# raulmur/ORB_SLAM2

Hardware: NVIDIA H100
Metric: stereo frames/sec (ORB extract L+R + ComputeStereoMatches, KITTI-shaped 1242x375 @2000 kpts) (higher is better)
Workload: dtype u8

## Files before the change

### orb_slam2_b200/csrc/k_fast.cu

```cuda
#include <cuda.h>

#include <cstring>

#include "borb_internal.h"

#include <algorithm>
#include <type_traits>
#include <vector>

namespace borb {

namespace {

constexpr int TP = 160;
constexpr int HB = FAST_H_BAND;
static_assert(HB >= 60 && HB <= 127, "a one-row band (hCell <= 59) must fit; collect packs the row into 7 bits");
constexpr int TROWS = HB + 6;
constexpr int QCAP = HB * 128;
constexpr int RG_MAX = (HB + 7) / 8;
constexpr int WSEG = RG_MAX * 32;
constexpr int RMAX = HB / 30;
constexpr int NCX = 128 / 30 + 1;
constexpr int SM_SCORE = TROWS * TP, SM_QUEUE = SM_SCORE + HB * TP, SM_WQUEUE = SM_QUEUE + QCAP * 2;
constexpr int FAST_SMEM = SM_WQUEUE + 8 * WSEG * 4;
static_assert(SM_SCORE % 16 == 0 && SM_WQUEUE % 4 == 0, "shared-memory carve-up alignment");

__device__ __forceinline__ uint32_t smem_u32(const void* p) { return (uint32_t)__cvta_generic_to_shared(p); }

template <int DX>
__device__ __forceinline__ uint32_t win(uint32_t W0, uint32_t W1, uint32_t W2) {
    if (DX == 0) return W1;
    if (DX > 0) return __byte_perm(W1, W2, DX | ((DX + 1) << 4) | ((DX + 2) << 8) | ((DX + 3) << 12));
    constexpr int K = 4 + DX;
    return __byte_perm(W0, W1, K | ((K + 1) << 4) | ((K + 2) << 8) | ((K + 3) << 12));
}

__device__ __forceinline__ uint32_t gt_flag(uint32_t q, uint32_t v, uint32_t K) {
    const uint32_t a = __vabsdiffu4(q, v);
    return (a + K) | a;
}

__device__ __forceinline__ uint32_t score_pair(const uint32_t (&d)[16], uint32_t v2) {
    uint32_t lo3[16], hi3[16];
#pragma unroll
    for (int k = 0; k < 16; k++) {
        lo3[k] = __vimin3_s16x2(d[k], d[(k + 1) & 15], d[(k + 2) & 15]);
        hi3[k] = __vimax3_s16x2(d[k], d[(k + 1) & 15], d[(k + 2) & 15]);
    }
    uint32_t lo9[16], hi9[16];
#pragma unroll
    for (int k = 0; k < 16; k++) {
        lo9[k] = __vimin3_s16x2(lo3[k], lo3[(k + 3) & 15], lo3[(k + 6) & 15]);
        hi9[k] = __vimax3_s16x2(hi3[k], hi3[(k + 3) & 15], hi3[(k + 6) & 15]);
    }
    uint32_t bb[5], dd[5];
#pragma unroll
    for (int k = 0; k < 5; k++) {
        bb[k] = __vimax3_s16x2(lo9[3 * k], lo9[3 * k + 1], lo9[3 * k + 2]);
        dd[k] = __vimin3_s16x2(hi9[3 * k], hi9[3 * k + 1], hi9[3 * k + 2]);
    }
    const uint32_t bright = __vimax3_s16x2(__vimax3_s16x2(bb[0], bb[1], bb[2]), __vimax3_s16x2(bb[3], bb[4], lo9[15]), bb[0]);
    const uint32_t darkm = __vimin3_s16x2(__vimin3_s16x2(dd[0], dd[1], dd[2]), __vimin3_s16x2(dd[3], dd[4], hi9[15]), dd[0]);
    return __viaddmax_s16x2_relu(__vmaxs2(__vsub2(bright, v2), __vsub2(v2, darkm)), 0xFFFFFFFFu, 0u);
}

__device__ __forceinline__ uint32_t score_pixels(const uint8_t* pa, const uint8_t* pb) {
    constexpr int RX[16] = {0, 1, 2, 3, 3, 3, 2, 1, 0, -1, -2, -3, -3, -3, -2, -1};
    constexpr int RY[16] = {3, 3, 2, 1, 0, -1, -2, -3, -3, -3, -2, -1, 0, 1, 2, 3};
    uint32_t d[16];
#pragma unroll
    for (int k = 0; k < 16; k++) {
        const int o = RY[k] * TP + RX[k];
        d[k] = (uint32_t)pa[o] | ((uint32_t)pb[o] << 16);
    }
    return score_pair(d, (uint32_t)pa[0] | ((uint32_t)pb[0] << 16));
}

}

struct TMaps { CUtensorMap m[BORB_MAX_LEVELS]; };

struct __align__(16) FastTile { int8_t l, ncell, rowsPerBlk, pad; int16_t x0, x1, y0, y1, wCell, hCell; };
static_assert(sizeof(FastTile) == 16, "one 16-byte load per CTA");

__global__ void __launch_bounds__(256, 4) fast_kernel(const __grid_constant__ Geometry g, const __grid_constant__ TMaps tm,
                                                   const FastTile* __restrict__ tiles, uint32_t* __restrict__ cand, int* __restrict__ cand_cnt) {
    extern __shared__ __align__(128) uint8_t smem[];
    uint8_t* tile = smem;
    uint8_t* score = smem + SM_SCORE;
    uint16_t* queue = reinterpret_cast<uint16_t*>(smem + SM_QUEUE);
    uint32_t* wqueue = reinterpret_cast<uint32_t*>(smem + SM_WQUEUE);
    __shared__ __align__(8) unsigned long long bar;
    __shared__ int pn, qn, needB;
    __shared__ int cellHasIni[RMAX * NCX];
    __shared__ uint8_t cellOf[128];
    __shared__ uint8_t rowOf[HB];

    const int img = blockIdx.y;
    const FastTile T = tiles[blockIdx.x];
    const int l = T.l, ncell = T.ncell, x0 = T.x0, x1 = T.x1, y0 = T.y0, y1 = T.y1;
    const int wCell = T.wCell, hCell = T.hCell;
    const LevelGeom& L = g.lv[l];
    const int tw = x1 - x0, th = y1 - y0;
    const int tid = threadIdx.x;
    const int lane = tid & 31, wrp = tid >> 5;

    const int xs = (x0 - 4) & ~15;
    const int off = x0 - xs;
    if (tid == 0) {
        asm volatile("mbarrier.init.shared::cta.b64 [%0], 1;" ::"r"(smem_u32(&bar)));
        asm volatile("fence.mbarrier_init.release.cluster;" ::: "memory");
        const uint32_t bytes = (uint32_t)TP * (uint32_t)fast_box_rows(T.rowsPerBlk, hCell);
        asm volatile("mbarrier.arrive.expect_tx.shared::cta.b64 _, [%0], %1;" ::"r"(smem_u32(&bar)), "r"(bytes) : "memory");
        asm volatile(
            "cp.async.bulk.tensor.3d.shared::cluster.global.tile.mbarrier::complete_tx::bytes [%0], [%1, {%2, %3, %4}], [%5];"
            ::"r"(smem_u32(tile)), "l"(reinterpret_cast<uint64_t>(&tm.m[l])), "r"(xs), "r"(y0 - 3), "r"(img), "r"(smem_u32(&bar))
            : "memory");
    }
    if (tid < RMAX * NCX) cellHasIni[tid] = 0;
    if (tid < 128) cellOf[tid] = (uint8_t)(tid / wCell);
    if (tid < HB) rowOf[tid] = (uint8_t)(tid / hCell);
    if (tid == 0) { pn = 0; qn = 0; needB = 0; }
    __syncthreads();
    asm volatile(
        "{\n"
        ".reg .pred p;\n"
        "FAST_TMA_WAIT:\n"
        "mbarrier.try_wait.parity.shared::cta.b64 p, [%0], 0;\n"
        "@p bra FAST_TMA_DONE;\n"
        "bra FAST_TMA_WAIT;\n"
        "FAST_TMA_DONE:\n"
        "}\n" ::"r"(smem_u32(&bar))
        : "memory");
    if (g.fast_mode == 1) {
        if (reinterpret_cast<const uint32_t*>(tile)[tid] == 0x12345678u && cand_cnt[0] == -1) cand[0] = 1;
        return;
    }

    const uint32_t* T32 = reinterpret_cast<const uint32_t*>(tile);
    uint32_t* S32 = reinterpret_cast<uint32_t*>(score);
    const int wbase = off >> 2;
    const int wc = wbase + lane;
    uint32_t vmask = 0;
#pragma unroll
    for (int b = 0; b < 4; b++)
        if (4 * wc + b - off >= 0 && 4 * wc + b - off < tw) vmask |= 0x80u << (8 * b);

    auto collect = [&](int t, const uint32_t (&mr)[RMAX], bool zero, auto banded) {
        constexpr bool BANDED = decltype(banded)::value;
        const uint32_t K = (uint32_t)(127 - min(t, 127)) * 0x01010101u;
        uint32_t mm[RMAX];
#pragma unroll
        for (int r = 0; r < (BANDED ? RMAX : 1); r++) {
            mm[r] = mr[r];
            asm volatile("" : "+r"(mm[r]));
        }
        const bool reject = t <= 127;
        const int RG = (th + 7) >> 3;
        const int yBeg = wrp * RG, yEnd = min(th, yBeg + RG);
        uint32_t a0[7], a1[7], a2[7];
        int wcount = 0;
        if (yBeg < yEnd) {
#pragma unroll
            for (int j = 0; j < 6; j++) {
                const uint32_t* rp = T32 + (yBeg + j) * (TP / 4) + wc - 1;
                a0[j] = rp[0]; a1[j] = rp[1]; a2[j] = rp[2];
            }
        }
        for (int it0 = 0; it0 < RG; it0 += 7)
#pragma unroll
        for (int it = 0; it < 7; it++) {
            const int yy = yBeg + it0 + it;
            if (yy < yEnd) {
                {
                    const uint32_t* rp = T32 + (yy + 6) * (TP / 4) + wc - 1;
                    a0[(it + 6) % 7] = rp[0]; a1[(it + 6) % 7] = rp[1]; a2[(it + 6) % 7] = rp[2];
                }
                uint32_t m = mm[0];
                if constexpr (BANDED) {
#pragma unroll
                    for (int r = 1; r < RMAX; r++)
                        if (yy >= r * hCell) m = mm[r];
                }
#define ROW(dy) a0[(it + (dy) + 3) % 7], a1[(it + (dy) + 3) % 7], a2[(it + (dy) + 3) % 7]
                uint32_t f = m;
                if (reject && m) {
                    const uint32_t v = a1[(it + 3) % 7];
                    uint32_t acc = gt_flag(win<0>(ROW(3)), v, K) | gt_flag(win<0>(ROW(-3)), v, K);
                    acc &= gt_flag(win<2>(ROW(2)), v, K) | gt_flag(win<-2>(ROW(-2)), v, K);
                    acc &= gt_flag(win<3>(ROW(0)), v, K) | gt_flag(win<-3>(ROW(0)), v, K);
                    acc &= gt_flag(win<2>(ROW(-2)), v, K) | gt_flag(win<-2>(ROW(2)), v, K);
                    f = acc & m;
                }
#undef ROW
                const unsigned bal = __ballot_sync(0xFFFFFFFFu, f != 0);
                if (zero && m != 0) S32[yy * (TP / 4) + wc] = 0;
                if (f) wqueue[wrp * WSEG + wcount + __popc(bal & ((1u << lane) - 1))] = f | (uint32_t)(yy << 8) | (uint32_t)wc;
                wcount += __popc(bal);
            }
        }
        __syncwarp();
        for (int i = 0; i < wcount; i += 32) {
            const uint32_t we = i + lane < wcount ? wqueue[wrp * WSEG + i + lane] : 0u;
            const uint32_t fl = we & 0x80808080u;
            const int c = __popc(fl);
            int incl = c;
#pragma unroll
            for (int o2 = 1; o2 < 32; o2 <<= 1) {
                const int s = __shfl_up_sync(0xFFFFFFFFu, incl, o2);
                if (lane >= o2) incl += s;
            }
            int base = 0;
            if (lane == 31) base = atomicAdd(&pn, incl);
            base = __shfl_sync(0xFFFFFFFFu, base, 31) + incl - c;
            const int e = (int)((we >> 8) & 127) << 8 | (int)(4 * (we & 127));
#pragma unroll
            for (int b = 0; b < 4; b++)
                if (fl & (0x80u << (8 * b))) queue[base++] = (uint16_t)(e + b);
        }
    };

    auto score_queue = [&](int t) {
        const int np = pn;
        const int tc = max(t, 1);
        for (int rb = 0; rb < np; rb += 512) {
            const int e0 = rb + wrp * 64 + lane, e1 = e0 + 32;
            const bool va = e0 < np, vb = e1 < np;
            const int qa = va ? queue[e0] : off;
            const int qb = vb ? queue[e1] : qa;
            __syncthreads();
            if (rb + wrp * 64 < np) {
                const int ia = (qa >> 8) * TP + (qa & 255), ib = (qb >> 8) * TP + (qb & 255);
                const uint32_t s2 = score_pixels(tile + ia + 3 * TP, tile + ib + 3 * TP);
                const int sa = (int)(s2 & 0xFFFFu), sb = (int)(s2 >> 16);
                if (va) score[ia] = (uint8_t)sa;
                if (vb) score[ib] = (uint8_t)sb;
                const bool ca = va && sa >= tc, cb = vb && sb >= tc;
                if (__any_sync(0xFFFFFFFFu, ca || cb)) {
                    const int c = (int)ca + (int)cb;
                    int incl = c;
#pragma unroll
                    for (int o2 = 1; o2 < 32; o2 <<= 1) {
                        const int s = __shfl_up_sync(0xFFFFFFFFu, incl, o2);
                        if (lane >= o2) incl += s;
                    }
                    int base = 0;
                    if (lane == 31) base = atomicAdd(&qn, incl);
                    base = __shfl_sync(0xFFFFFFFFu, base, 31) + incl - c;
                    if (ca) queue[base++] = (uint16_t)qa;
                    if (cb) queue[base] = (uint16_t)qb;
                }
            }
        }
    };

    {
        const uint32_t mA[RMAX] = {vmask};
        collect(g.ini_th, mA, true, std::false_type());
    }
    __syncthreads();
    if (g.fast_mode == 2) {
        if (pn == -1) cand[0] = 1;
        return;
    }
    score_queue(g.ini_th);
    __syncthreads();
    int nq = qn;
    if (g.fast_mode == 3) {
        if (nq == -1) cand[0] = 1;
        return;
    }

    uint32_t* out = cand + (size_t)img * g.cand_image_stride + L.cand_off;
    int* cnt = cand_cnt + img * g.nlevels + l;

    auto nms = [&](int n, bool mark) {
        for (int e = tid; e < n; e += 256) {
            const int q = queue[e];
            const int col = q & 255, yy = q >> 8;
            const int xx = col - off;
            const int s = score[yy * TP + col];
            const int c = cellOf[xx], r = rowOf[yy];
            const int cx0 = c * wCell, cx1 = min(cx0 + wCell, tw);
            const int cy0 = r * hCell, cy1 = min(cy0 + hCell, th);
            bool ismax = true;
#pragma unroll
            for (int dy = -1; dy <= 1; dy++)
#pragma unroll
                for (int dx = -1; dx <= 1; dx++) {
                    if (dx == 0 && dy == 0) continue;
                    const int qx = xx + dx, qy = yy + dy;
                    if (qx < cx0 || qx >= cx1 || qy < cy0 || qy >= cy1) continue;
                    if (!(s > (int)score[qy * TP + col + dx])) ismax = false;
                }
            if (ismax) {
                if (mark) cellHasIni[r * NCX + c] = 1;
            } else
                queue[e] = 0xFFFF;
        }
    };
    auto emit = [&](int n) {
        for (int eb = 0; eb < n; eb += 256) {
            const int e = eb + tid;
            int s = 0, xx = 0, yy = 0;
            if (e < n) {
                const int q = queue[e];
                if (q != 0xFFFF) {
                    const int col = q & 255;
                    yy = q >> 8; xx = col - off;
                    s = score[yy * TP + col];
                }
            }
            const unsigned m = __ballot_sync(0xFFFFFFFFu, s > 0);
            if (m) {
                int base = 0;
                if (lane == 0) base = atomicAdd(cnt, __popc(m));
                base = __shfl_sync(0xFFFFFFFFu, base, 0);
                if (s > 0) {
                    const int pos = base + __popc(m & ((1u << lane) - 1));
                    if (pos < L.cand_cap) out[pos] = pack_xys(x0 + xx, y0 + yy, s);
                }
            }
        }
    };

    nms(nq, true);
    __syncthreads();
    emit(nq);
    if (tid < RMAX * NCX) {
        const int r = tid / NCX, c = tid - r * NCX;
        if (r * hCell < th && c < ncell && c * wCell < tw && !cellHasIni[tid] && g.min_th < g.ini_th) needB = 1;
    }
    __syncthreads();
    if (!needB) return;

    {
        uint32_t need[RMAX];
#pragma unroll
        for (int r = 0; r < RMAX; r++) {
            need[r] = 0;
#pragma unroll
            for (int b = 0; b < 4; b++) {
                const int xx = 4 * wc + b - off;
                if (xx >= 0 && xx < tw && !cellHasIni[r * NCX + cellOf[xx]]) need[r] |= 0x80u << (8 * b);
            }
        }
        if (tid == 0) { pn = 0; qn = 0; }
        __syncthreads();
        collect(g.min_th, need, false, std::true_type());
        __syncthreads();
        score_queue(g.min_th);
        __syncthreads();
        nq = qn;
        nms(nq, false);
        __syncthreads();
        emit(nq);
    }
}

typedef CUresult (*EncodeTiledFn)(CUtensorMap*, CUtensorMapDataType, cuuint32_t, void*, const cuuint64_t*, const cuuint64_t*,
                                  const cuuint32_t*, const cuuint32_t*, CUtensorMapInterleave, CUtensorMapSwizzle,
                                  CUtensorMapL2promotion, CUtensorMapFloatOOBfill);

borb_status build_fast_tmaps(const Geometry& g, const Workspace& ws, void* out_tmaps) {
    static EncodeTiledFn encode = nullptr;
    if (!encode) {
        void* fn = nullptr;
        cudaDriverEntryPointQueryResult qres;
        cudaError_t e = cudaGetDriverEntryPoint("cuTensorMapEncodeTiled", &fn, cudaEnableDefault, &qres);
        if (e != cudaSuccess || qres != cudaDriverEntryPointSuccess || !fn) {
            set_error("cuTensorMapEncodeTiled unavailable (%s)", cudaGetErrorString(e));
            return BORB_ERR_CUDA;
        }
        encode = (EncodeTiledFn)fn;
    }
    TMaps* tm = reinterpret_cast<TMaps*>(out_tmaps);
    std::memset(tm, 0, sizeof(TMaps));
    for (int l = 0; l < g.nlevels; l++) {
        const LevelGeom& L = g.lv[l];
        cuuint64_t dims[3] = {(cuuint64_t)L.w, (cuuint64_t)L.h, (cuuint64_t)ws.max_images};
        cuuint64_t strides[2] = {(cuuint64_t)L.pitch, (cuuint64_t)g.pyr_image_stride};
        cuuint32_t box[3] = {(cuuint32_t)TP, (cuuint32_t)fast_box_rows(L.rowsPerBlk, L.hCell), 1};
        cuuint32_t estr[3] = {1, 1, 1};
        CUresult r = encode(&tm->m[l], CU_TENSOR_MAP_DATA_TYPE_UINT8, 3, ws.pyr + L.pyr_off, dims, strides, box, estr,
                            CU_TENSOR_MAP_INTERLEAVE_NONE, CU_TENSOR_MAP_SWIZZLE_NONE, CU_TENSOR_MAP_L2_PROMOTION_L2_128B,
                            CU_TENSOR_MAP_FLOAT_OOB_FILL_NONE);
        if (r != CUDA_SUCCESS) {
            set_error("cuTensorMapEncodeTiled failed for level %d (CUresult %d)", l, (int)r);
            return BORB_ERR_CUDA;
        }
    }
    return BORB_OK;
}

size_t fast_tmaps_bytes() { return sizeof(TMaps); }

borb_status build_fast_tiles(const Geometry& g, Workspace& ws) {
    std::vector<FastTile> t;
    for (int l = 0; l < g.nlevels; l++) {
        const LevelGeom& L = g.lv[l];
        for (int cellRow = 0; cellRow < L.nRows; cellRow += L.rowsPerBlk)
            for (int blkCol = 0; blkCol < L.blkCols; blkCol++) {
                const int cell0 = blkCol * L.cellsPerBlk;
                const int ncell = std::min(L.cellsPerBlk, L.nCols - cell0);
                const int nrow = std::min(L.rowsPerBlk, L.nRows - cellRow);
                const int x0 = EDGE + cell0 * L.wCell, x1 = std::min(x0 + ncell * L.wCell, L.w - EDGE);
                const int y0 = EDGE + cellRow * L.hCell, y1 = std::min(y0 + nrow * L.hCell, L.h - EDGE);
                if (x0 >= x1 || y0 >= y1) continue;
                FastTile f;
                f.l = (int8_t)l; f.ncell = (int8_t)ncell; f.rowsPerBlk = (int8_t)L.rowsPerBlk; f.pad = 0;
                f.x0 = (int16_t)x0; f.x1 = (int16_t)x1; f.y0 = (int16_t)y0; f.y1 = (int16_t)y1;
                f.wCell = (int16_t)L.wCell; f.hCell = (int16_t)L.hCell;
                t.push_back(f);
            }
    }
    cudaFree(ws.fast_tiles); ws.fast_tiles = nullptr;
    ws.fast_n_tiles = (int)t.size();
    if (t.empty()) return BORB_OK;
    BORB_CUDA(cudaMalloc(&ws.fast_tiles, t.size() * sizeof(FastTile)));
    BORB_CUDA(cudaMemcpy(ws.fast_tiles, t.data(), t.size() * sizeof(FastTile), cudaMemcpyHostToDevice));
    return BORB_OK;
}

int launch_fast(const Geometry& g, const Workspace& ws, int n_images, cudaStream_t s) {
    if (ws.fast_n_tiles == 0) return 0;
    allow_max_smem((const void*)fast_kernel);
    dim3 grid(ws.fast_n_tiles, n_images);
    fast_kernel<<<grid, 256, FAST_SMEM, s>>>(g, *reinterpret_cast<const TMaps*>(ws.fast_tmaps), reinterpret_cast<const FastTile*>(ws.fast_tiles), ws.cand, ws.cand_cnt);
    return 1;
}

}
```

Before: 44120.

## Process two FAST rows per step, warp-skip empty bands, fuse NMS and emit

The FAST collect loop now handles two rows per iteration in the unbanded pass and writes paired queue entries with 8-byte stores. The banded pass skips rows where no lane has a live mask. The score buffer is zeroed up front with vector stores, replacing the per-row zeroing inside collect. NMS now counts the survivors it keeps, so emit needs only one warp-level atomic per warp and drops one block barrier. In exchange it uses more registers and a larger wqueue segment, and emit now relies on each warp's NMS and emit covering the same entries.

Result: faster. 45390 (median of 6 runs) (+2.9%).

```diff
diff --git a/orb_slam2_b200/csrc/k_fast.cu b/orb_slam2_b200/csrc/k_fast.cu
--- a/orb_slam2_b200/csrc/k_fast.cu
+++ b/orb_slam2_b200/csrc/k_fast.cu
@@ -18,12 +18,12 @@
 constexpr int TROWS = HB + 6;
 constexpr int QCAP = HB * 128;
 constexpr int RG_MAX = (HB + 7) / 8;
-constexpr int WSEG = RG_MAX * 32;
+constexpr int WSEG = (RG_MAX + 1) / 2 * 64;
 constexpr int RMAX = HB / 30;
 constexpr int NCX = 128 / 30 + 1;
 constexpr int SM_SCORE = TROWS * TP, SM_QUEUE = SM_SCORE + HB * TP, SM_WQUEUE = SM_QUEUE + QCAP * 2;
 constexpr int FAST_SMEM = SM_WQUEUE + 8 * WSEG * 4;
-static_assert(SM_SCORE % 16 == 0 && SM_WQUEUE % 4 == 0, "shared-memory carve-up alignment");
+static_assert(SM_SCORE % 16 == 0 && SM_WQUEUE % 8 == 0 && WSEG % 2 == 0, "shared-memory carve-up alignment");
 
 __device__ __forceinline__ uint32_t smem_u32(const void* p) { return (uint32_t)__cvta_generic_to_shared(p); }
 
@@ -121,6 +121,7 @@
     if (tid < 128) cellOf[tid] = (uint8_t)(tid / wCell);
     if (tid < HB) rowOf[tid] = (uint8_t)(tid / hCell);
     if (tid == 0) { pn = 0; qn = 0; needB = 0; }
+    for (int i = tid; i < th * (TP / 16); i += 256) reinterpret_cast<uint4*>(score)[i] = make_uint4(0u, 0u, 0u, 0u);
     __syncthreads();
     asm volatile(
         "{\n"
@@ -138,7 +139,6 @@
     }
 
     const uint32_t* T32 = reinterpret_cast<const uint32_t*>(tile);
-    uint32_t* S32 = reinterpret_cast<uint32_t*>(score);
     const int wbase = off >> 2;
     const int wc = wbase + lane;
     uint32_t vmask = 0;
@@ -146,7 +146,7 @@
     for (int b = 0; b < 4; b++)
         if (4 * wc + b - off >= 0 && 4 * wc + b - off < tw) vmask |= 0x80u << (8 * b);
 
-    auto collect = [&](int t, const uint32_t (&mr)[RMAX], bool zero, auto banded) {
+    auto collect = [&](int t, const uint32_t (&mr)[RMAX], auto banded) {
         constexpr bool BANDED = decltype(banded)::value;
         const uint32_t K = (uint32_t)(127 - min(t, 127)) * 0x01010101u;
         uint32_t mm[RMAX];
@@ -155,10 +155,10 @@
             mm[r] = mr[r];
             asm volatile("" : "+r"(mm[r]));
         }
-        const bool reject = t <= 127;
         const int RG = (th + 7) >> 3;
         const int yBeg = wrp * RG, yEnd = min(th, yBeg + RG);
-        uint32_t a0[7], a1[7], a2[7];
+        constexpr int NR = BANDED ? 1 : 2, NW = NR + 6;
+        uint32_t a0[NW], a1[NW], a2[NW];
         int wcount = 0;
         if (yBeg < yEnd) {
 #pragma unroll
@@ -167,36 +167,51 @@
                 a0[j] = rp[0]; a1[j] = rp[1]; a2[j] = rp[2];
             }
         }
-        for (int it0 = 0; it0 < RG; it0 += 7)
-#pragma unroll
-        for (int it = 0; it < 7; it++) {
+        for (int it0 = 0; it0 < RG; it0 += NW)
+#pragma unroll
+        for (int it = 0; it < NW; it += NR) {
             const int yy = yBeg + it0 + it;
             if (yy < yEnd) {
-                {
-                    const uint32_t* rp = T32 + (yy + 6) * (TP / 4) + wc - 1;
-                    a0[(it + 6) % 7] = rp[0]; a1[(it + 6) % 7] = rp[1]; a2[(it + 6) % 7] = rp[2];
+                uint32_t m[NR], f[NR], e[NR];
+#pragma unroll
+                for (int k = 0; k < NR; k++) {
+                    const bool live = k == 0 || yy + k < yEnd;
+                    if (live) {
+                        const uint32_t* rp = T32 + (yy + 6 + k) * (TP / 4) + wc - 1;
+                        a0[(it + 6 + k) % NW] = rp[0]; a1[(it + 6 + k) % NW] = rp[1]; a2[(it + 6 + k) % NW] = rp[2];
+                    }
+                    m[k] = mm[0];
+                    if constexpr (BANDED) {
+#pragma unroll
+                        for (int r = 1; r < RMAX; r++)
+                            if (yy + k >= r * hCell) m[k] = mm[r];
+                    }
+                    if (!live) m[k] = 0;
                 }
-                uint32_t m = mm[0];
-                if constexpr (BANDED) {
-#pragma unroll
-                    for (int r = 1; r < RMAX; r++)
-                        if (yy >= r * hCell) m = mm[r];
-                }
-#define ROW(dy) a0[(it + (dy) + 3) % 7], a1[(it + (dy) + 3) % 7], a2[(it + (dy) + 3) % 7]
-                uint32_t f = m;
-                if (reject && m) {
-                    const uint32_t v = a1[(it + 3) % 7];
-                    uint32_t acc = gt_flag(win<0>(ROW(3)), v, K) | gt_flag(win<0>(ROW(-3)), v, K);
+                if (BANDED && !__any_sync(0xFFFFFFFFu, m[0] != 0)) continue;
+#define ROW(dy) a0[(c + (dy)) % NW], a1[(c + (dy)) % NW], a2[(c + (dy)) % NW]
+#pragma unroll
+                for (int k = 0; k < NR; k++) {
+                    const int c = it + 3 + k;
+                    const uint32_t v = a1[c % NW];
+                    uint32_t acc = m[k] & (gt_flag(win<0>(ROW(3)), v, K) | gt_flag(win<0>(ROW(-3)), v, K));
                     acc &= gt_flag(win<2>(ROW(2)), v, K) | gt_flag(win<-2>(ROW(-2)), v, K);
                     acc &= gt_flag(win<3>(ROW(0)), v, K) | gt_flag(win<-3>(ROW(0)), v, K);
                     acc &= gt_flag(win<2>(ROW(-2)), v, K) | gt_flag(win<-2>(ROW(2)), v, K);
-                    f = acc & m;
+                    f[k] = acc;
+                    e[k] = acc | (uint32_t)((yy + k) << 8) | (uint32_t)wc;
                 }
 #undef ROW
-                const unsigned bal = __ballot_sync(0xFFFFFFFFu, f != 0);
-                if (zero && m != 0) S32[yy * (TP / 4) + wc] = 0;
-                if (f) wqueue[wrp * WSEG + wcount + __popc(bal & ((1u << lane) - 1))] = f | (uint32_t)(yy << 8) | (uint32_t)wc;
-                wcount += __popc(bal);
+                const unsigned lt = (1u << lane) - 1;
+                if constexpr (NR == 1) {
+                    const unsigned bal = __ballot_sync(0xFFFFFFFFu, f[0] != 0);
+                    if (f[0]) wqueue[wrp * WSEG + wcount + __popc(bal & lt)] = e[0];
+                    wcount += __popc(bal);
+                } else {
+                    const unsigned bal = __ballot_sync(0xFFFFFFFFu, (f[0] | f[1]) != 0);
+                    if (f[0] | f[1]) *reinterpret_cast<uint2*>(&wqueue[wrp * WSEG + wcount + 2 * __popc(bal & lt)]) = make_uint2(e[0], e[1]);
+                    wcount += 2 * __popc(bal);
+                }
             }
         }
         __syncwarp();
@@ -256,7 +271,7 @@
 
     {
         const uint32_t mA[RMAX] = {vmask};
-        collect(g.ini_th, mA, true, std::false_type());
+        collect(g.ini_th, mA, std::false_type());
     }
     __syncthreads();
     if (g.fast_mode == 2) {
@@ -275,6 +290,7 @@
     int* cnt = cand_cnt + img * g.nlevels + l;
 
     auto nms = [&](int n, bool mark) {
+        int kept = 0;
         for (int e = tid; e < n; e += 256) {
             const int q = queue[e];
             const int col = q & 255, yy = q >> 8;
@@ -294,39 +310,35 @@
                     if (!(s > (int)score[qy * TP + col + dx])) ismax = false;
                 }
             if (ismax) {
+                kept++;
                 if (mark) cellHasIni[r * NCX + c] = 1;
             } else
                 queue[e] = 0xFFFF;
         }
+        return kept;
     };
-    auto emit = [&](int n) {
+    auto emit = [&](int n, int kept) {
+        const int total = __reduce_add_sync(0xFFFFFFFFu, kept);
+        if (total == 0) return;
+        int base = 0;
+        if (lane == 0) base = atomicAdd(cnt, total);
+        base = __shfl_sync(0xFFFFFFFFu, base, 0);
+        const unsigned lt = (1u << lane) - 1;
         for (int eb = 0; eb < n; eb += 256) {
             const int e = eb + tid;
-            int s = 0, xx = 0, yy = 0;
-            if (e < n) {
-                const int q = queue[e];
-                if (q != 0xFFFF) {
-                    const int col = q & 255;
-                    yy = q >> 8; xx = col - off;
-                    s = score[yy * TP + col];
-                }
-            }
-            const unsigned m = __ballot_sync(0xFFFFFFFFu, s > 0);
-            if (m) {
-                int base = 0;
-                if (lane == 0) base = atomicAdd(cnt, __popc(m));
-                base = __shfl_sync(0xFFFFFFFFu, base, 0);
-                if (s > 0) {
-                    const int pos = base + __popc(m & ((1u << lane) - 1));
-                    if (pos < L.cand_cap) out[pos] = pack_xys(x0 + xx, y0 + yy, s);
-                }
-            }
+            const int q = e < n ? queue[e] : 0xFFFF;
+            const unsigned m = __ballot_sync(0xFFFFFFFFu, q != 0xFFFF);
+            if (q != 0xFFFF) {
+                const int col = q & 255, yy = q >> 8;
+                const int pos = base + __popc(m & lt);
+                if (pos < L.cand_cap) out[pos] = pack_xys(x0 + col - off, y0 + yy, score[yy * TP + col]);
+            }
+            base += __popc(m);
         }
     };
 
-    nms(nq, true);
+    emit(nq, nms(nq, true));
     __syncthreads();
-    emit(nq);
     if (tid < RMAX * NCX) {
         const int r = tid / NCX, c = tid - r * NCX;
         if (r * hCell < th && c < ncell && c * wCell < tw && !cellHasIni[tid] && g.min_th < g.ini_th) needB = 1;
@@ -347,14 +359,12 @@
         }
         if (tid == 0) { pn = 0; qn = 0; }
         __syncthreads();
-        collect(g.min_th, need, false, std::true_type());
+        collect(g.min_th, need, std::true_type());
         __syncthreads();
         score_queue(g.min_th);
         __syncthreads();
         nq = qn;
-        nms(nq, false);
-        __syncthreads();
-        emit(nq);
+        emit(nq, nms(nq, false));
     }
 }
 
```
